# JackAILab/ConsistentID

Hardware: AMD Instinct MI355X
Metric: 512x512 SD1.5 images/sec/node @50 DDIM steps (higher is better)
Workload: dtype f16; 1 GPU; sd15 ConsistentID 512x512, 50 DDIM steps, batch 4/GPU (global 4), CFG batch 8, LoRA rank 128 merged, start_merge_step 30, hipGraph on; global_batch=4, parallelism=dp1 (images sharded, no in-step collective)

## Files before the change

### consistentid_amd/csrc/gemm.hip

```cpp
#include "xattn_core.h"
#include "gemm_args.h"
#include "../../include/cid.h"

#ifndef CID_HALO_STAGGER
#define CID_HALO_STAGGER 1
#endif
#ifdef CID_CONV_TRACE
__device__ unsigned long long g_conv_trace[2 * 4096];
#define CONV_STAMP(k) do { if (tr_on) tr_ts[k] = __builtin_readcyclecounter(); } while (0)
#define CONV_FLUSH() do { if (tr_on && lane == 0 && tr_n + 8 <= 4096) { for (int q_ = 0; q_ < 8; ++q_) g_conv_trace[tr_slot * 4096 + tr_n + q_] = tr_ts[q_]; } tr_n += 8; } while (0)
#else
#define CONV_STAMP(k) do { } while (0)
#define CONV_FLUSH() do { } while (0)
#endif
#if defined(CID_GEMM_ABLATION)
#define CID_ABL(bit) ((a.ablate & (bit)) != 0)
#else
#define CID_ABL(bit) false
#endif

namespace {
using cidg::GemmArgs;
using cidg::wait_vmcnt;

template <int N>
__device__ __forceinline__ void frags_landed(half8 (&f)[N]) {
#pragma unroll
    for (int i = 0; i < N; ++i) asm volatile("" : "+v"(f[i]));
}


constexpr int BK = 64;

typedef float f32x4v __attribute__((ext_vector_type(4)));

CID_DEVINL f32x4v mfma16(half8 a, half8 b, f32x4v c) {
    return __builtin_amdgcn_mfma_f32_16x16x32_f16(a, b, c, 0, 0, 0);
}

CID_DEVINL int swz_key(int r) { return ((r >> 1) & 3) << 1; }
CID_DEVINL int lds_off(int r, int c) { return r * 128 + ((c ^ swz_key(r)) << 4); }

CID_DEVINL float row16_sum(float v) {
#define CID_ROR(N) v += __builtin_bit_cast(float, __builtin_amdgcn_update_dpp(0, __builtin_bit_cast(int, v), 0x120 + N, 0xf, 0xf, false))
    CID_ROR(8); CID_ROR(4); CID_ROR(2); CID_ROR(1);
#undef CID_ROR
    return v;
}

template <int TM, int TN, bool VMODE, bool LN, bool NLOOP = false, bool ACT = false>
CID_DEVINL void igemm_epilogue(const GemmArgs& a, f32x4v (&acc)[TM][TN], int m0, int n0, int wm, int wn,
                               int l16, int lq, char* smem, int wave, const float (&lmean)[TM], const float (&lrstd)[TM],
                               int nwaves, int wn_count, const half4 (&rpre)[TM][TN], bool rpre_valid) {
    if constexpr (VMODE) {
#pragma unroll
        for (int c = 0; c < TN; ++c) {
            const int n = n0 + (wn * TN + c) * 16 + l16;
            if (n >= a.n_end) continue;
            const int cg = n - a.n_vt0;
            const int head = cg / a.dhead, dd = cg - head * a.dhead;
            const float bv = LN ? a.ln_b[n] : (a.bias ? (float)a.bias[n] : 0.f);
            const float sv = LN ? a.ln_s[n] : 0.f;
#pragma unroll
            for (int t = 0; t < TM; ++t) {
                const int mt = m0 + (wm * TM + t) * 16;
                if (mt >= a.M) continue;
                const int b = mt / a.ntok, tok0 = mt - b * a.ntok;
                half_t* dst = a.vt + ((long)(b * a.heads + head) * a.dvp + dd) * a.ntok + tok0;
                half4 o;
                if constexpr (LN) {
#pragma unroll
                    for (int i = 0; i < 4; ++i) {
                        const float mu = __shfl(lmean[t], 4 * lq + i, 64), rs = __shfl(lrstd[t], 4 * lq + i, 64);
                        o[i] = (half_t)(rs * (acc[t][c][i] - mu * sv) + bv);
                    }
                } else {
#pragma unroll
                    for (int i = 0; i < 4; ++i) o[i] = (half_t)(acc[t][c][i] + bv);
                }
                *reinterpret_cast<half4*>(dst + 8 * (lq & 1) + 4 * (lq >> 1)) = o;
            }
        }
        return;
    } else {
        if (!NLOOP && a.splitk > 1) {
            float* wsp = a.ws + (long)blockIdx.z * a.M * a.N;
#pragma unroll
            for (int t = 0; t < TM; ++t) {
                const int m = m0 + (wm * TM + t) * 16 + l16;
                if (m >= a.M) continue;
#pragma unroll
                for (int c = 0; c < TN; ++c) {
                    const int n = n0 + (wn * TN + c) * 16 + 4 * lq;
                    if (n >= a.n_end) continue;
                    *reinterpret_cast<f32x4v*>(wsp + (long)m * a.N + n) = acc[t][c];
                }
            }
            return;
        }
        if (NLOOP || a.mode == 1) {
#pragma unroll
            for (int c = 0; c + 1 < TN; c += 2) {
                const int nt = n0 + (wn * TN + c) * 16;
                if (nt >= a.n_end) continue;
                float bv[4] = {0.f, 0.f, 0.f, 0.f}, bg[4] = {0.f, 0.f, 0.f, 0.f};
                float sv[4] = {0.f, 0.f, 0.f, 0.f}, sg[4] = {0.f, 0.f, 0.f, 0.f};
                if constexpr (LN) {
                    const f32x4v fv = *reinterpret_cast<const f32x4v*>(a.ln_b + nt + 4 * lq);
                    const f32x4v fg = *reinterpret_cast<const f32x4v*>(a.ln_b + nt + 16 + 4 * lq);
                    const f32x4v qv = *reinterpret_cast<const f32x4v*>(a.ln_s + nt + 4 * lq);
                    const f32x4v qg = *reinterpret_cast<const f32x4v*>(a.ln_s + nt + 16 + 4 * lq);
#pragma unroll
                    for (int i = 0; i < 4; ++i) { bv[i] = fv[i]; bg[i] = fg[i]; sv[i] = qv[i]; sg[i] = qg[i]; }
                } else if (a.bias && !CID_ABL(512)) {
                    const half4 hv = *reinterpret_cast<const half4*>(a.bias + nt + 4 * lq);
                    const half4 hg = *reinterpret_cast<const half4*>(a.bias + nt + 16 + 4 * lq);
// ... 78 lines not shown
                }
                if constexpr (ACT) {
#pragma unroll
                    for (int i = 0; i < 4; ++i) v[i] = __builtin_fmaxf(v[i], 0.f);
                }
                half4 o;
#pragma unroll
                for (int i = 0; i < 4; ++i) o[i] = (half_t)v[i];
                *reinterpret_cast<half4*>(stg + (t * 16 + l16) * P + c * 16 + 4 * lq) = o;
                if (gstat && mok) {
#pragma unroll
                    for (int i = 0; i < 4; ++i) { const float f = (float)o[i]; gs[c][i] += f; gq[c][i] = __builtin_fmaf(f, f, gq[c][i]); }
                }
            }
        }
        float* gst = reinterpret_cast<float*>(smem + nwaves * (TM * 16 * P) * 2);
        if (gstat) {
#pragma unroll
            for (int c = 0; c < TN; ++c)
#pragma unroll
                for (int i = 0; i < 4; ++i) { gs[c][i] = row16_sum(gs[c][i]); gq[c][i] = row16_sum(gq[c][i]); }
            if (l16 == 0) {
#pragma unroll
                for (int c = 0; c < TN; ++c)
#pragma unroll
                    for (int i = 0; i < 4; ++i) {
                        float* p = gst + (wave * (TN * 16) + c * 16 + 4 * lq + i) * 2;
                        p[0] = gs[c][i]; p[1] = gq[c][i];
                    }
            }
        }
        asm volatile("s_waitcnt lgkmcnt(0)" ::: "memory");
        constexpr int CPR = TN * 2;
        constexpr int PER = TM * 16 * CPR / 64;
        static_assert((TM * 16 * CPR) % 64 == 0, "tile chunks must divide over the wave");
        const int lane = lq * 16 + l16;
#pragma unroll
        for (int i = 0; i < PER; ++i) {
            const int e = i * 64 + lane;
            const int r = e / CPR, ch = e - r * CPR;
            const int m = m0 + wm * TM * 16 + r;
            const int n = n0 + wn * TN * 16 + ch * 8;
            const half8 val = *reinterpret_cast<const half8*>(stg + r * P + ch * 8);
            if (m < a.M && n < a.n_end) {
                *reinterpret_cast<half8*>(a.out + (long)m * a.ldo + n) = val;
                if (a.out2) *reinterpret_cast<half8*>(a.out2 + (long)m * a.ldo + n) = val;
            }
        }
        if (gstat) {
            __builtin_amdgcn_s_barrier();
            const int bn = wn_count * TN * 16, wm_count = nwaves / wn_count;
            const int nu = bn / a.gn_unit;
            const int u = wave * 64 + lq * 16 + l16;
            if (u < nu && n0 + u * a.gn_unit < a.n_end) {
                float S = 0.f, Q = 0.f;
                for (int w_ = 0; w_ < wm_count; ++w_)
                    for (int ch = u * a.gn_unit; ch < (u + 1) * a.gn_unit; ++ch) {
                        const int wv = w_ * wn_count + ch / (TN * 16);
                        const float* p = gst + (wv * (TN * 16) + ch % (TN * 16)) * 2;
                        S += p[0]; Q += p[1];
                    }
                float* dst = a.gn_stats + ((long)(m0 / (wm_count * TM * 16)) * (a.N / a.gn_unit) + (n0 - a.n_begin) / a.gn_unit + u) * 2;
                dst[0] = S; dst[1] = Q;
            }
        }
    }
}

template <int TM, int TN>
CID_DEVINL bool prefetch_residual(const GemmArgs& a, half4 (&rpre)[TM][TN], int m0, int n0, int wm, int wn, int l16, int lq) {
    const bool on = TM >= 4 && a.res != nullptr && a.mode == 0 && a.splitk == 1;
    if constexpr (TM < 4) return false;
#pragma unroll
    for (int t = 0; t < TM; ++t)
#pragma unroll
        for (int c = 0; c < TN; ++c) {
            const int m = m0 + (wm * TM + t) * 16 + l16, n = n0 + (wn * TN + c) * 16 + 4 * lq;
            half4 z = {(half_t)0.f, (half_t)0.f, (half_t)0.f, (half_t)0.f};
            rpre[t][c] = (on && m < a.M && n < a.n_end) ? *reinterpret_cast<const half4*>(a.res + (long)m * a.ldr + n) : z;
        }
    return on;
}

template <int TM, int TN, int WM, int WN, bool VMODE, int NBUF, bool LN, bool NLOOP = false, int ATT_D = 0, bool ACT = false>
__global__ void __launch_bounds__(64 * WM * WN, (NLOOP && TM == 2) ? 4 : 2)
igemm_kernel(GemmArgs a) {
#if defined(__HIP_DEVICE_COMPILE__)
    constexpr int NW = WM * WN;
    constexpr int BM = 16 * TM * WM;
    constexpr int BN = 16 * TN * WN;
    constexpr int XPW = (BM / 8 + NW - 1) / NW, WPW = (BN / 8 + NW - 1) / NW;
    constexpr int XI = XPW * NW, WI = WPW * NW;
    constexpr int XBYTES = XI * 1024, WBYTES = BN * 128;
    constexpr int SBYTES = XBYTES + WBYTES;
    extern __shared__ __attribute__((aligned(16))) char smem[];
    typedef __attribute__((address_space(3))) void lds_void;

    const int tid = threadIdx.x;
    const int lane = tid & 63;
    const int wave = __builtin_amdgcn_readfirstlane(tid >> 6);
    const int l16 = lane & 15, lq = lane >> 4;
    const int r8 = lane >> 3, c8 = lane & 7;
    const int wm = wave / WN, wn = wave % WN;
    int nb_, mb_;
    cidg::xcd_tile(a, nb_, mb_);
    const int n0 = a.n_begin + nb_ * BN * a.nloop;
    const int m0 = mb_ * BM;

    constexpr unsigned OOB = 0x80000000u;
    const __amdgpu_buffer_rsrc_t rs_x1 = __builtin_amdgcn_make_buffer_rsrc((void*)a.x1, 0, a.bytes_x1, 0x00020000);
    const __amdgpu_buffer_rsrc_t rs_x2 = __builtin_amdgcn_make_buffer_rsrc((void*)(a.x2 ? a.x2 : a.x1), 0,
                                                                           a.x2 ? a.bytes_x2 : 0, 0x00020000);
    const __amdgpu_buffer_rsrc_t rs_w = __builtin_amdgcn_make_buffer_rsrc((void*)a.w, 0, a.bytes_w, 0x00020000);
    int xb[XPW], xy[XPW], xx[XPW], xsw[XPW];
    bool xok[XPW];
#pragma unroll
    for (int j = 0; j < XPW; ++j) {
        const int R = (j * NW + wave) * 8 + r8;
        const int m = m0 + R;
        xok[j] = (R < BM) && (m < a.M);
        xsw[j] = (c8 ^ swz_key(R)) * 8;
        if (a.taps == 9) {
            const int hw = a.Ho * a.Wo;
            const int b = m / hw, rem = m - b * hw;
            xb[j] = b; xy[j] = rem / a.Wo; xx[j] = rem - xy[j] * a.Wo;
        } else {
            xb[j] = 0; xy[j] = 0; xx[j] = m;
        }
    }
    unsigned woff[WPW];
#pragma unroll
    for (int j = 0; j < WPW; ++j) {
        const int R = (j * NW + wave) * 8 + r8;
        const bool ok = (R < BN) && (n0 + R < a.n_end);
        woff[j] = ok ? (unsigned)(((long)(n0 + R) * a.ktot + (c8 ^ swz_key(R)) * 8) * 2) : OOB;
    }
    unsigned xoff1[XPW], xoff2[XPW];
    auto set_tap = [&](int tap) {
        const int dy = (a.taps == 9) ? tap / 3 + a.tap0 : 0;
        const int dx = (a.taps == 9) ? tap - (tap / 3) * 3 + a.tap0 : 0;
#pragma unroll
        for (int j = 0; j < XPW; ++j) {
            bool ok = xok[j];
            long row = xx[j];
            if (a.taps == 9) {
                int yy = xy[j] * a.stride + dy, xs = xx[j] * a.stride + dx;
                const int Hv = a.Hi << a.up, Wv = a.Wi << a.up;
                ok = ok && (yy >= 0) && (yy < Hv) && (xs >= 0) && (xs < Wv);
                yy >>= a.up; xs >>= a.up;
                row = ((long)xb[j] * a.Hi + yy) * a.Wi + xs;
            }
            xoff1[j] = ok ? (unsigned)((row * a.ld1 + xsw[j]) * 2) : OOB;
            xoff2[j] = ok ? (unsigned)((row * a.ld2 + xsw[j]) * 2) : OOB;
        }
    };
    int ld_tap = -1;

    auto issue = [&](int slab, int buf, unsigned wtile = 0u) {
        const int cs = slab / a.taps;
        const int tap = slab - cs * a.taps;
        const int cbase = cs * BK;
        if (tap != ld_tap) { set_tap(tap); ld_tap = tap; }
        char* xs = smem + buf * SBYTES;
        char* ws = xs + XBYTES;
        const bool first = cbase < a.c1;
        const unsigned coff = (unsigned)((first ? cbase : cbase - a.c1) * 2);
        if (first) {
#pragma unroll
            for (int j = 0; j < XPW; ++j)
                __builtin_amdgcn_raw_ptr_buffer_load_lds(rs_x1, (lds_void*)(xs + (j * NW + wave) * 1024), 16, xoff1[j] + coff, 0, 0, 0);
        } else {
#pragma unroll
            for (int j = 0; j < XPW; ++j)
                __builtin_amdgcn_raw_ptr_buffer_load_lds(rs_x2, (lds_void*)(xs + (j * NW + wave) * 1024), 16, xoff2[j] + coff, 0, 0, 0);
        }
        const unsigned koff = (unsigned)((tap * (a.c1 + a.c2) + cbase) * 2) + wtile;
#pragma unroll
        for (int j = 0; j < WPW; ++j)
            if ((j + 1) * NW * 8 <= BN || (j * NW + wave) * 8 < BN)
                __builtin_amdgcn_raw_ptr_buffer_load_lds(rs_w, (lds_void*)(ws + (j * NW + wave) * 1024), 16, woff[j] + koff, 0, 0, 0);
    };

    f32x4v acc[TM][TN];
#pragma unroll
    for (int t = 0; t < TM; ++t)
#pragma unroll
        for (int c = 0; c < TN; ++c) acc[t][c] = f32x4v{0.f, 0.f, 0.f, 0.f};

    const int s_begin = (int)((long)a.nslab * blockIdx.z / a.splitk);
    const int s_end = (int)((long)a.nslab * (blockIdx.z + 1) / a.splitk);

    static_assert(NBUF >= 2 && NBUF <= 4, "two to four LDS stages");
    auto read_frags = [&](const char* xs, const char* ws, int ks, half8 (&xf)[TM], half8 (&wf)[TN]) {
        if (CID_ABL(256)) return;
#pragma unroll
        for (int t = 0; t < TM; ++t)
            xf[t] = *reinterpret_cast<const half8*>(xs + lds_off((wm * TM + t) * 16 + l16, ks * 4 + lq));
#pragma unroll
        for (int c = 0; c < TN; ++c)
            wf[c] = *reinterpret_cast<const half8*>(ws + lds_off((wn * TN + c) * 16 + l16, ks * 4 + lq));
    };
    auto mma = [&](const half8 (&xf)[TM], const half8 (&wf)[TN]) {
#pragma unroll
        for (int t = 0; t < TM; ++t)
#pragma unroll
            for (int c = 0; c < TN; ++c)
                acc[t][c] = VMODE ? mfma16(xf[t], wf[c], acc[t][c]) : mfma16(wf[c], xf[t], acc[t][c]);
    };

    float lsum[TM], lsq[TM];
    half2v lpiv[TM];
#pragma unroll
    for (int t = 0; t < TM; ++t) {
        lsum[t] = 0.f; lsq[t] = 0.f;
        half_t p = (half_t)0.f;
        if constexpr (LN) {
            const int row = m0 + (wm * TM + t) * 16 + l16;
            if (row < a.M) p = a.x1[(long)row * a.ld1];
        }
        lpiv[t] = half2v{p, p};
    }
    bool ln_on = true;
    auto ln_acc = [&](const half8 (&xf)[TM]) {
        if constexpr (LN) {
            if (!ln_on) return;
            const half2v one = {(half_t)1.f, (half_t)1.f};
#pragma unroll
            for (int t = 0; t < TM; ++t)
#pragma unroll
                for (int j = 0; j < 4; ++j) {
                    const half2v h = half2v{xf[t][2 * j], xf[t][2 * j + 1]} - lpiv[t];
                    lsum[t] = __builtin_amdgcn_fdot2(h, one, lsum[t], false);
                    lsq[t] = __builtin_amdgcn_fdot2(h, h, lsq[t], false);
                }
        }
    };

    float lmean[TM], lrstd[TM];
    auto ln_finish = [&]() {
#pragma unroll
        for (int t = 0; t < TM; ++t) {
            if constexpr (LN) {
                float sm = lsum[t], sq = lsq[t];
                sm += __shfl_xor(sm, 16, 64); sq += __shfl_xor(sq, 16, 64);
                sm += __shfl_xor(sm, 32, 64); sq += __shfl_xor(sq, 32, 64);
                const float inv = 1.f / (float)a.ktot;
                const float md = sm * inv;
                lmean[t] = (float)lpiv[t][0] + md;
                lrstd[t] = sq == 0.f ? 0.f : rsqrtf(fmaxf(sq * inv - md * md, 0.f) + a.ln_eps);
            } else { lmean[t] = 0.f; lrstd[t] = 1.f; }
        }
    };

    half4 rpre[TM][TN];
    const bool rpre_valid = VMODE ? false : prefetch_residual<TM, TN>(a, rpre, m0, n0, wm, wn, l16, lq);
    if constexpr (NLOOP) {
        static_assert(NBUF == 2, "the N-loop form runs on two stages");
        const int ns = a.nslab, T = ns * a.nloop;
        const unsigned wstep = (unsigned)((long)BN * a.ktot * 2);
        int is_ks = 0; unsigned is_w = 0u;
        set_tap(0);
        auto issue_next = [&](int buf) {
            char* xs = smem + buf * SBYTES;
            char* ws = xs + XBYTES;
            const unsigned coff = (unsigned)(is_ks * BK * 2);
#pragma unroll
            for (int j = 0; j < XPW; ++j)
                __builtin_amdgcn_raw_ptr_buffer_load_lds(rs_x1, (lds_void*)(xs + (j * NW + wave) * 1024), 16, xoff1[j] + coff, 0, 0, 0);
#pragma unroll
            for (int j = 0; j < WPW; ++j)
                __builtin_amdgcn_raw_ptr_buffer_load_lds(rs_w, (lds_void*)(ws + (j * NW + wave) * 1024), 16, woff[j] + coff + is_w, 0, 0, 0);
            if (++is_ks == ns) { is_ks = 0; is_w += wstep; }
        };
        half8 xf0[TM], wf0[TN], xf1[TM], wf1[TN];
        issue_next(0);
        asm volatile("s_waitcnt vmcnt(0)" ::: "memory");
        __builtin_amdgcn_s_barrier();
        read_frags(smem, smem + XBYTES, 0, xf0, wf0);
        if (1 < T) issue_next(1);
        frags_landed(xf0); frags_landed(wf0);
        int cur = 0, ks = 0, nt = 0;
        for (int f = 0; f < T; ++f) {
            const char* xs = smem + cur * SBYTES;
            read_frags(xs, xs + XBYTES, 1, xf1, wf1);
            mma(xf0, wf0);
            ln_acc(xf0);
            __builtin_amdgcn_sched_barrier(0);
            frags_landed(xf1); frags_landed(wf1);
            if (f + 1 < T) {
                asm volatile("s_waitcnt vmcnt(0) lgkmcnt(0)" ::: "memory");
                __builtin_amdgcn_s_barrier();
                if (f + 2 < T) issue_next(cur);
                const char* xn = smem + (cur ^ 1) * SBYTES;
                read_frags(xn, xn + XBYTES, 0, xf0, wf0);
            }
            mma(xf1, wf1);
            ln_acc(xf1);
            __builtin_amdgcn_sched_barrier(0);
            frags_landed(xf0); frags_landed(wf0);
            cur ^= 1;
            if (++ks == ns) {
                if (nt == 0) { ln_finish(); ln_on = false; }
                igemm_epilogue<TM, TN, false, LN, true>(a, acc, m0, n0 + nt * BN, wm, wn, l16, lq, smem, wave, lmean, lrstd, NW, WN, rpre, false);
#pragma unroll
                for (int t = 0; t < TM; ++t)
#pragma unroll
                    for (int c = 0; c < TN; ++c) acc[t][c] = f32x4v{0.f, 0.f, 0.f, 0.f};
                ks = 0; ++nt;
                __builtin_amdgcn_sched_barrier(0);
            }
        }
        asm volatile("s_waitcnt vmcnt(0)" ::: "memory");
        return;
    }
    {
    int pw = XPW;
#pragma unroll
    for (int j = 0; j < WPW; ++j)
        if ((j + 1) * NW * 8 <= BN || (j * NW + wave) * 8 < BN) ++pw;
    half8 xf0[TM], wf0[TN], xf1[TM], wf1[TN];
    const int nsl = s_end - s_begin;
    int pre = 0;
    if (!CID_ABL(128))
        for (; pre < NBUF - 1 && pre < nsl; ++pre) issue(s_begin + pre, pre);
    if (NBUF == 2) asm volatile("s_waitcnt vmcnt(0)" ::: "memory");
    else wait_vmcnt((pre > 0 ? pre - 1 : 0) * pw);
    __builtin_amdgcn_s_barrier();
    read_frags(smem, smem + XBYTES, 0, xf0, wf0);
    if (NBUF - 1 < nsl && !CID_ABL(1)) issue(s_begin + NBUF - 1, NBUF - 1);
    frags_landed(xf0); frags_landed(wf0);

    int cur = 0;
    for (int slab = s_begin; slab < s_end; ++slab) {
        const char* xs = smem + cur * SBYTES;
        const int nxt = (cur + 1 == NBUF) ? 0 : cur + 1;
        read_frags(xs, xs + XBYTES, 1, xf1, wf1);
        if (!CID_ABL(2)) mma(xf0, wf0);
        ln_acc(xf0);
        __builtin_amdgcn_sched_barrier(0);
        frags_landed(xf1); frags_landed(wf1);
        if (slab + 1 < s_end) {
            if (NBUF == 2) asm volatile("s_waitcnt vmcnt(0) lgkmcnt(0)" ::: "memory");
            else {
                int young = s_end - 2 - slab;
                if (young > NBUF - 2) young = NBUF - 2;
                if (young < 0 || CID_ABL(1)) young = 0;
                wait_vmcnt(young * pw);
                asm volatile("s_waitcnt lgkmcnt(0)" ::: "memory");
            }
            __builtin_amdgcn_s_barrier();
            if (slab + NBUF < s_end && !CID_ABL(1)) issue(slab + NBUF, cur);
            const char* xn = smem + nxt * SBYTES;
            read_frags(xn, xn + XBYTES, 0, xf0, wf0);
        }
        if (!CID_ABL(2)) mma(xf1, wf1);
        ln_acc(xf1);
        __builtin_amdgcn_sched_barrier(0);
        frags_landed(xf0); frags_landed(wf0);
        cur = nxt;
    }
    }
    asm volatile("s_waitcnt vmcnt(0)" ::: "memory");
    ln_finish();

    static_assert(NW * TM * 16 * (TN * 16 + 8) * 2 + NW * TN * 16 * 8 <= NBUF * SBYTES, "epilogue staging fits the pipeline stages");
    if constexpr (ATT_D > 0) {
        static_assert(!VMODE && !NLOOP && BN % ATT_D == 0 && BM % 32 == 0, "the tile spans whole heads and 32-token groups");
        constexpr int TP = BN + 8;
        static_assert(BM * TP * 2 <= NBUF * SBYTES, "the Q / O tile fits the pipeline stages");
        half_t* T = reinterpret_cast<half_t*>(smem);
        __builtin_amdgcn_s_barrier();
#pragma unroll
        for (int t = 0; t < TM; ++t)
#pragma unroll
            for (int c = 0; c < TN; ++c) {
                const int nl = (wn * TN + c) * 16 + 4 * lq;
                float v[4];
#pragma unroll
                for (int i = 0; i < 4; ++i) v[i] = acc[t][c][i];
                if constexpr (LN) {
                    const f32x4v qs = *reinterpret_cast<const f32x4v*>(a.ln_s + n0 + nl);
                    const f32x4v qb = *reinterpret_cast<const f32x4v*>(a.ln_b + n0 + nl);
#pragma unroll
                    for (int i = 0; i < 4; ++i) v[i] = lrstd[t] * (v[i] - lmean[t] * qs[i]) + qb[i];
                }
                half4 o;
#pragma unroll
                for (int i = 0; i < 4; ++i) o[i] = (half_t)v[i];
                *reinterpret_cast<half4*>(T + ((wm * TM + t) * 16 + l16) * TP + nl) = o;
            }
        asm volatile("s_waitcnt lgkmcnt(0)" ::: "memory");
        __builtin_amdgcn_s_barrier();
        {
            const int idx = lane & 31, hi = lane >> 5;
            const long row = a.att_kvrow[m0 / a.ntok];
            constexpr int QKS = (ATT_D + 15) / 16, DVT = (ATT_D + 31) / 32;
            constexpr int NHL = BN / ATT_D, NTG = BM / 32;
            const int h0 = n0 / ATT_D;
            for (int u = wave; u < NHL * NTG; u += NW) {
                const int hl = u / NTG, tg = u - hl * NTG;
                const half_t* kph = a.att_kp + row * a.att_krow + (long)(h0 + hl) * XC_KTILES * QKS * 512 + lane * 8;
                const half_t* vph = a.att_vp + row * a.att_vrow + (long)(h0 + hl) * DVT * XC_PV_KSTEPS * 512 + lane * 8;
                xattn_core_unit<ATT_D, 1, true>(T, TP, tg * 32, hl * ATT_D, kph, vph, a.att_n_txt, a.att_n_ip, a.att_scale, idx, hi);
            }
        }
        asm volatile("s_waitcnt lgkmcnt(0)" ::: "memory");
        __builtin_amdgcn_s_barrier();
        constexpr int CPR = BN / 8;
        for (int e = tid; e < BM * CPR; e += 64 * NW) {
            const int r = e / CPR, cc = e - r * CPR;
            if (m0 + r < a.M)
                *reinterpret_cast<half8*>(a.out + (long)(m0 + r) * a.ldo + n0 + cc * 8) = *reinterpret_cast<const half8*>(T + r * TP + cc * 8);
        }
        return;
    }
    igemm_epilogue<TM, TN, VMODE, LN, false, ACT>(a, acc, m0, n0, wm, wn, l16, lq, smem, wave, lmean, lrstd, NW, WN, rpre, rpre_valid);
#endif
}

template <int TM, int TN, int WM, int WN>
__global__ void __launch_bounds__(64 * WM * WN, 2)
igemm_halo_kernel(GemmArgs a) {
#if defined(__HIP_DEVICE_COMPILE__)
    constexpr int NW = WM * WN;
    constexpr int BM = 16 * TM * WM;
    constexpr int BN = 16 * TN * WN;
    constexpr int HPW = 7;
    constexpr int HROWS = HPW * NW * 8;
    constexpr int WPW = (BN / 8 + NW - 1) / NW;
    constexpr int HBYTES = HROWS * 128, WBYTES = WPW * NW * 1024;
    extern __shared__ __attribute__((aligned(16))) char smem[];
    typedef __attribute__((address_space(3))) void lds_void;
    char* hbuf = smem;
    char* wbuf = smem + 2 * HBYTES;

    const int tid = threadIdx.x;
    const int lane = tid & 63;
    const int wave = __builtin_amdgcn_readfirstlane(tid >> 6);
    const int l16 = lane & 15, lq = lane >> 4;
    const int r8 = lane >> 3, c8 = lane & 7;
    const int wm = wave / WN, wn = wave % WN;
    int nb_, mb_;
    cidg::xcd_tile(a, nb_, mb_);
    const int n0 = a.n_begin + nb_ * BN;
    const int m0 = mb_ * BM;

    const int W = a.Wo, H = a.Ho, HW = H * W;
    const int seg_tok = BM < HW ? BM : HW;
    const int rs = seg_tok / W;
    const int hs = (rs + 2) * (W + 2);
    const int nh = (BM / seg_tok) * hs;
    const int img0 = m0 / HW;
    const int y0 = (m0 - img0 * HW) / W;

    constexpr unsigned OOB = 0x80000000u;
    const __amdgpu_buffer_rsrc_t rs_x1 = __builtin_amdgcn_make_buffer_rsrc((void*)a.x1, 0, a.bytes_x1, 0x00020000);
    const __amdgpu_buffer_rsrc_t rs_x2 = __builtin_amdgcn_make_buffer_rsrc((void*)(a.x2 ? a.x2 : a.x1), 0,
                                                                           a.x2 ? a.bytes_x2 : 0, 0x00020000);
    const __amdgpu_buffer_rsrc_t rs_w = __builtin_amdgcn_make_buffer_rsrc((void*)a.w, 0, a.bytes_w, 0x00020000);

    unsigned hoff1[HPW], hoff2[HPW];
#pragma unroll
    for (int j = 0; j < HPW; ++j) {
        const int hr = (j * NW + wave) * 8 + r8;
        const int seg = hr / hs, rem = hr - seg * hs;
        const int hy = rem / (W + 2), hx = rem - hy * (W + 2);
        const int img = img0 + seg;
        const int yy = y0 + hy - 1, xx = hx - 1;
        const bool ok = (hr < nh) && (yy >= 0) && (yy < H) && (xx >= 0) && (xx < W) && ((long)img * HW < a.M);
        const long row = ((long)img * H + yy) * W + xx;
        const int swz = (c8 ^ swz_key(hr)) * 8;
        hoff1[j] = ok ? (unsigned)((row * a.ld1 + swz) * 2) : OOB;
        hoff2[j] = ok ? (unsigned)((row * a.ld2 + swz) * 2) : OOB;
    }
    unsigned woff[WPW];
#pragma unroll
    for (int j = 0; j < WPW; ++j) {
        const int R = (j * NW + wave) * 8 + r8;
        const bool ok = (R < BN) && (n0 + R < a.n_end);
        woff[j] = ok ? (unsigned)(((long)(n0 + R) * a.ktot + (c8 ^ swz_key(R)) * 8) * 2) : OOB;
    }
    int hbase[TM];
#pragma unroll
    for (int t = 0; t < TM; ++t) {
        const int ml = (wm * TM + t) * 16 + l16;
        const int seg = ml / seg_tok, rem = ml - seg * seg_tok;
        const int y = rem / W, x = rem - y * W;
        hbase[t] = seg * hs + (y + 1) * (W + 2) + (x + 1);
        asm volatile("" : "+v"(hbase[t]));
    }

    const int ctot = a.c1 + a.c2;
    auto issue_halo = [&](int cs, int hb) {
        const int cbase = cs * BK;
        char* dst = hbuf + hb * HBYTES;
        if (cbase < a.c1) {
#pragma unroll
            for (int j = 0; j < HPW; ++j)
                if ((j * NW + wave) * 8 < nh)
                    __builtin_amdgcn_raw_ptr_buffer_load_lds(rs_x1, (lds_void*)(dst + (j * NW + wave) * 1024), 16, hoff1[j] + cbase * 2, 0, 0, 0);
// ... 226 lines not shown
        *reinterpret_cast<half4*>(a.out + (long)m * a.ldo + n) = o;
        if (a.out2) *reinterpret_cast<half4*>(a.out2 + (long)m * a.ldo + n) = o;
    }
}

template <int TM, int TN, int WM, int WN, bool VMODE, bool LN, bool NLOOP = false, int NBUF = 2, int ATT_D = 0, bool ACT = false>
int launch_one_ln(const GemmArgs& a, int ncols, hipStream_t s) {
    constexpr int BM = 16 * TM * WM, BN = 16 * TN * WN;
    constexpr int NW = WM * WN;
    constexpr int STAGE = ((BM / 8 + NW - 1) / NW) * NW * 1024 + BN * 128;
    constexpr int SMEM = NBUF * STAGE;
    static_assert(SMEM <= 160 * 1024, "LDS budget");
    auto kern = igemm_kernel<TM, TN, WM, WN, VMODE, NBUF, LN, NLOOP, ATT_D, ACT>;
    static bool configured = false;
    if (!configured) {
        hipError_t herr = hipFuncSetAttribute((const void*)kern, hipFuncAttributeMaxDynamicSharedMemorySize, SMEM);
        if (herr != hipSuccess) {
            cid_set_error("cid_gemm_f16: cannot reserve %d bytes of LDS (%s)", SMEM, hipGetErrorString(herr));
            return -5;
        }
        configured = true;
    }
    dim3 grid((ncols + BN - 1) / BN / (NLOOP ? a.nloop : 1), (a.M + BM - 1) / BM, VMODE ? 1 : a.splitk);
    GemmArgs b = a;
    b.xcd_pn = cidg::choose_xcd_pn((int)grid.x, (int)grid.y, 2.0 * ncols * a.ktot, (double)a.bytes_x1 + a.bytes_x2);
    hipLaunchKernelGGL(kern, grid, dim3(64 * WM * WN), SMEM, s, b);
    return 0;
}

template <int TM, int TN, int WM, int WN, bool VMODE>
int launch_one(const GemmArgs& a, int ncols, hipStream_t s) {
    if constexpr (!VMODE && TN == 4 && WM * WN == 8) {
        if (a.nloop > 1)
            return a.ln_s ? launch_one_ln<TM, TN, WM, WN, false, true, true>(a, ncols, s)
                          : launch_one_ln<TM, TN, WM, WN, false, false, true>(a, ncols, s);
    }
    if constexpr (!VMODE && TN == 5) {
        if (a.nbuf == 3)
            return a.ln_s ? launch_one_ln<TM, TN, WM, WN, false, true, false, 3>(a, ncols, s)
                          : launch_one_ln<TM, TN, WM, WN, false, false, false, 3>(a, ncols, s);
    }
    return a.ln_s ? launch_one_ln<TM, TN, WM, WN, VMODE, true>(a, ncols, s) : launch_one_ln<TM, TN, WM, WN, VMODE, false>(a, ncols, s);
}

template <int TM, int TN, int WM, int WN, int ATT_D>
int launch_att(const GemmArgs& a, hipStream_t s) {
    return a.ln_s ? launch_one_ln<TM, TN, WM, WN, false, true, false, 2, ATT_D>(a, a.N, s)
                  : launch_one_ln<TM, TN, WM, WN, false, false, false, 2, ATT_D>(a, a.N, s);
}

template <int TM, int TN, int WM, int WN>
int launch_act(const GemmArgs& a, hipStream_t s) {
    return launch_one_ln<TM, TN, WM, WN, false, false, false, 2, 0, true>(a, a.N, s);
}

void launch_splitk_epilogue(const GemmArgs& a, hipStream_t s) {
    const long items = (long)a.M * (a.N >> 2);
    const int grid = (int)((items + 255) / 256 > 2048 ? 2048 : (items + 255) / 256);
    hipLaunchKernelGGL(splitk_epilogue_kernel, dim3(grid), dim3(256), 0, s, a);
}

template <int TM, int TN, int WM, int WN>
int launch_halo(GemmArgs a, hipStream_t s) {
    constexpr int BM = 16 * TM * WM, BN = 16 * TN * WN, NW = WM * WN;
    constexpr int SMEM = 2 * (7 * NW * 1024) + 2 * (((BN / 8 + NW - 1) / NW) * NW * 1024);
    static_assert(SMEM <= 160 * 1024, "LDS budget");
    auto kern = igemm_halo_kernel<TM, TN, WM, WN>;
    static bool configured = false;
    if (!configured) {
        hipError_t herr = hipFuncSetAttribute((const void*)kern, hipFuncAttributeMaxDynamicSharedMemorySize, SMEM);
        if (herr != hipSuccess) {
            cid_set_error("cid_gemm_f16: cannot reserve %d bytes of LDS (%s)", SMEM, hipGetErrorString(herr));
            return -5;
        }
        configured = true;
    }
    dim3 grid((a.N + BN - 1) / BN, (a.M + BM - 1) / BM, a.splitk);
    a.xcd_pn = cidg::choose_xcd_pn((int)grid.x, (int)grid.y, 2.0 * a.N * a.ktot, (double)a.bytes_x1 + a.bytes_x2);
    hipLaunchKernelGGL(kern, grid, dim3(64 * NW), SMEM, s, a);
    if (a.splitk > 1) launch_splitk_epilogue(a, s);
    return 0;
}

template <int TM, int TN, int WM, int WN>
int launch(GemmArgs a, hipStream_t s) {
    const int n_plain = (a.mode == 2) ? a.n_vt0 : a.N;
    a.n_begin = 0; a.n_end = n_plain;
    int rc = launch_one<TM, TN, WM, WN, false>(a, n_plain, s);
    if (rc) return rc;
    if (a.splitk > 1) launch_splitk_epilogue(a, s);
    if (a.mode == 2 && a.N > a.n_vt0) {
        GemmArgs v = a;
        v.n_begin = a.n_vt0; v.n_end = a.N; v.splitk = 1;
        rc = launch_one<TM, TN, WM, WN, true>(v, a.N - a.n_vt0, s);
    }
    return rc;
}

}

extern "C" int cid_gemm_f16(const cid_gemm_desc* d, cid_stream_t stream) {
    using namespace cidg;
    GemmPlan p;
    int rc = plan(d, p);
    if (rc) return rc;
    const GemmArgs& a = p.a;
    hipStream_t s = (hipStream_t)stream;
    switch (p.family) {
        case CID_GEMM_FAMILY_GEGLU_H32:
            rc = launch_geglu_h32(a, s);
            break;
        case CID_GEMM_FAMILY_IGEMM_ATT:
            if (p.cfg == G128x128) rc = launch_att<2, 4, 4, 2, 64>(a, s);
            else if (p.cfg == B128x160) rc = a.dhead == 80 ? launch_att<2, 5, 4, 2, 80>(a, s) : launch_att<2, 5, 4, 2, 160>(a, s);
            else rc = a.dhead == 80 ? launch_att<2, 5, 2, 2, 80>(a, s) : launch_att<2, 5, 2, 2, 160>(a, s);
            break;
        case CID_GEMM_FAMILY_CONV_H32:
        case CID_GEMM_FAMILY_CONV_H32_PHASE:
            rc = launch_conv_h32(a, p.bm, s);
            break;
        case CID_GEMM_FAMILY_IGEMM_HALO:
            rc = launch_halo<4, 5, 4, 2>(a, s);
            break;
        default:
            if (p.act) {
                switch (p.cfg) {
                    case A256x160: rc = launch_act<4, 5, 4, 2>(a, s); break;
                    case B128x160: rc = launch_act<2, 5, 4, 2>(a, s); break;
                    case C64x160:  rc = launch_act<2, 5, 2, 2>(a, s); break;
                    case G256x128: rc = launch_act<4, 4, 4, 2>(a, s); break;
                    case G128x128: rc = launch_act<2, 4, 4, 2>(a, s); break;
                    case O64x64:   rc = launch_act<2, 2, 2, 2>(a, s); break;
                    case O128x32:  rc = launch_act<2, 2, 4, 1>(a, s); break;
                }
            } else {
                switch (p.cfg) {
                    case A256x160: rc = launch<4, 5, 4, 2>(a, s); break;
                    case B128x160: rc = launch<2, 5, 4, 2>(a, s); break;
                    case C64x160:  rc = launch<2, 5, 2, 2>(a, s); break;
                    case G256x128: rc = launch<4, 4, 4, 2>(a, s); break;
                    case G128x128: rc = launch<2, 4, 4, 2>(a, s); break;
                    case O64x64:   rc = launch<2, 2, 2, 2>(a, s); break;
                    case O128x32:  rc = launch<2, 2, 4, 1>(a, s); break;
                }
            }
            break;
    }
    if (rc) return rc;
    CID_CHECK_LAUNCH("cid_gemm_f16");
    return 0;
}
```

### consistentid_amd/csrc/gemm_args.h

```cpp
#pragma once
#include "common.h"

struct cid_gemm_desc;

namespace cidg {

struct GemmArgs {
    const half_t* x1; const half_t* x2;
    int c1, c2, ld1, ld2;
    const half_t* w;
    half_t* out; int ldo;
    half_t* out2;
    const half_t* bias;
    const half_t* rowbias; int ld_rowbias; int rows_per_sample;
    const half_t* res; int ldr;
    int M, N, taps;
    int Hi, Wi, Ho, Wo, stride, up;
    int mode;
    half_t* vt; int n_vt0, heads, dhead, dvp, ntok;
    int n_begin, n_end;
    int ktot;
    int nslab;
    int cslabs;
    int splitk;
    int nloop;
    int nbuf;
    const half_t* att_kp; const half_t* att_vp; const int* att_kvrow;
    long att_krow, att_vrow;
    int att_n_txt, att_n_ip;
    float att_scale;
    unsigned bytes_x1, bytes_x2, bytes_w;
    float* ws;
    const float* ln_s;
    const float* ln_b;
    float ln_eps;
    float* gn_stats;
    int gn_unit;
    int ablate;
    int xcd_pn;
    int tap0;
    const half_t* w4;
};

CID_DEVINL void xcd_tile(const GemmArgs& a, int& nb, int& mb) {
    const int gx = gridDim.x, gy = gridDim.y;
    int bid = blockIdx.y * gx + blockIdx.x;
    if (a.xcd_pn > 0) {
        const int pn = a.xcd_pn;
        const int x = bid & 7, l = bid >> 3;
        const int bnc = gx / pn;
        nb = (x % pn) * bnc + l % bnc;
        mb = (x / pn) * (gy * pn >> 3) + l / bnc;
    } else {
        const int nwg = gx * gy;
        if ((nwg & 7) == 0) bid = (bid & 7) * (nwg >> 3) + (bid >> 3);
        nb = bid % gx;
        mb = bid / gx;
    }
}

int choose_xcd_pn(int gx, int gy, double w_bytes, double x_bytes);

enum TileCfg { A256x160, B128x160, C64x160, G256x128, G128x128, O64x64, O128x32 };
struct GemmPlan {
    GemmArgs a;
    TileCfg cfg;
    int bm, bn;
    int family;
    bool ln, act, vmode;
    bool sk_epilogue;
    int stats_rows;
};
int plan(const cid_gemm_desc* d, GemmPlan& p);

CID_DEVINL void wait_vmcnt(int n) {
#define CID_VM(N) case N: asm volatile("s_waitcnt vmcnt(" #N ")" ::: "memory"); break;
    switch (n) {
        CID_VM(0) CID_VM(1) CID_VM(2) CID_VM(3) CID_VM(4) CID_VM(5) CID_VM(6) CID_VM(7) CID_VM(8) CID_VM(9)
        CID_VM(10) CID_VM(11) CID_VM(12) CID_VM(13) CID_VM(14) CID_VM(15) CID_VM(16) CID_VM(17) CID_VM(18)
        CID_VM(19) CID_VM(20) CID_VM(21) CID_VM(22) CID_VM(23) CID_VM(24) CID_VM(25) CID_VM(26) CID_VM(27)
        CID_VM(28) CID_VM(29) CID_VM(30) CID_VM(31) CID_VM(32)
        default: asm volatile("s_waitcnt vmcnt(0)" ::: "memory"); break;
    }
#undef CID_VM
}

int launch_conv_h32(const GemmArgs& a, int bm, hipStream_t s);

int launch_geglu_h32(const GemmArgs& a, hipStream_t s);

}
```

### consistentid_amd/csrc/gemm_plan.hip

```cpp
#include "gemm_args.h"
#include "../../include/cid.h"
#include <stdlib.h>

namespace {
using namespace cidg;

int env_int(const char* name, int dflt) { const char* e = getenv(name); return e ? atoi(e) : dflt; }

struct PlanSwitches {
    int geglu_tile = env_int("CID_GEGLU_TILE", 0);
    int gemm_tile = env_int("CID_GEMM_TILE", 0);
    int gemm_sk = env_int("CID_GEMM_SK", 0);
    int prefer128 = env_int("CID_GEMM_PREFER128", 1);
    int geglu_nloop = env_int("CID_GEGLU_NLOOP", 0);
    int geglu_h32 = env_int("CID_GEGLU_H32", 1);
    int nbuf = env_int("CID_GEMM_NBUF", 0);
    int no_halo = env_int("CID_GEMM_NOHALO", 0);
    int conv_h32 = env_int("CID_CONV_H32", 1);
    int upconv_fold = env_int("CID_UPCONV_FOLD", 1);
    int xcd_2d = env_int("CID_XCD_2D", 1);
    int ablate = env_int("CID_GEMM_ABLATE", 0);
};

const PlanSwitches& switches() { static const PlanSwitches s; return s; }

constexpr int BK = 64;
constexpr long TARGET = 2048;

void set_tile(GemmPlan& p, TileCfg cfg) {
    static const int bm[] = { 256, 128, 64, 256, 128, 64, 128 }, bn[] = { 160, 160, 160, 128, 128, 64, 32 };
    p.cfg = cfg; p.bm = bm[cfg]; p.bn = bn[cfg];
}

int n_plain(const cid_gemm_desc* d) { return d->mode == 2 ? d->n_vt0 : d->N; }

long waves(const cid_gemm_desc* d, int bm, int bn, int w) { return (long)((d->M + bm - 1) / bm) * ((n_plain(d) + bn - 1) / bn) * w; }

int check_args(const cid_gemm_desc* d, GemmPlan& p) {
    CID_CHECK_ARG(d && d->x1 && d->w && d->out, "cid_gemm_f16: null pointer");
    CID_CHECK_ARG(d->taps == 1 || d->taps == 9, "cid_gemm_f16: taps must be 1 or 9 (got %d)", d->taps);
    CID_CHECK_ARG(d->c1 > 0 && d->c1 % 32 == 0 && d->c2 >= 0 && d->c2 % 32 == 0 && (d->c1 + d->c2) % 64 == 0 &&
                  (d->c2 == 0 || d->c1 % 64 == 0),
                  "cid_gemm_f16: channel counts must be multiples of 64 (c1=%d c2=%d)", d->c1, d->c2);
    CID_CHECK_ARG(d->c2 == 0 || d->x2, "cid_gemm_f16: c2 > 0 needs x2");
    CID_CHECK_ARG(d->N > 0 && d->N % 32 == 0 && d->M > 0, "cid_gemm_f16: bad M/N (%d, %d)", d->M, d->N);
    CID_CHECK_ARG(d->mode >= 0 && d->mode <= 3, "cid_gemm_f16: bad mode %d", d->mode);
    CID_CHECK_ARG(d->ld1 % 8 == 0 && d->ldo % 8 == 0 && (d->c2 == 0 || d->ld2 % 8 == 0) && (!d->res || d->ldr % 8 == 0),
                  "cid_gemm_f16: row pitches (ld1, ld2, ldo, ldr) must keep 16-byte alignment");
    CID_CHECK_ARG((((uintptr_t)d->out | (uintptr_t)d->res | (uintptr_t)d->out2) & 15) == 0,
                  "cid_gemm_f16: out / out2 / res must be 16-byte aligned (rows are stored and the residual is read in 16-byte chunks)");
    CID_CHECK_ARG((d->ln_s == nullptr) == (d->ln_b == nullptr), "cid_gemm_f16: ln_s and ln_b come together");
    CID_CHECK_ARG(!d->ln_s || (d->taps == 1 && d->c2 == 0 && !d->bias && d->ln_eps > 0.f),
                  "cid_gemm_f16: the LayerNorm fold applies to one-source linears; the bias belongs in ln_b");
    CID_CHECK_ARG(!d->out2 || d->mode == 0, "cid_gemm_f16: out2 (a second destination) goes with the plain epilogue, mode 0");
    const long rows_in = (d->taps == 9) ? (long)(d->M / (d->Ho * d->Wo)) * d->Hi * d->Wi : (long)d->M;
    const long b1 = ((rows_in - 1) * d->ld1 + d->c1) * 2, b2 = d->c2 ? ((rows_in - 1) * d->ld2 + d->c2) * 2 : 0;
    const long bw = (long)d->N * d->taps * (d->c1 + d->c2) * 2;
    CID_CHECK_ARG(b1 < 0x7fffffffL && b2 < 0x7fffffffL && bw < 0x7fffffffL, "cid_gemm_f16: tensor exceeds 2 GiB");
    p.a.bytes_x1 = (unsigned)b1; p.a.bytes_x2 = (unsigned)b2; p.a.bytes_w = (unsigned)bw;
    if (d->taps == 9) {
        CID_CHECK_ARG(d->Hi > 0 && d->Wi > 0 && d->Ho > 0 && d->Wo > 0 && (d->stride == 1 || d->stride == 2)
                      && (d->up == 0 || d->up == 1), "cid_gemm_f16: bad conv geometry");
        CID_CHECK_ARG(d->M % (d->Ho * d->Wo) == 0, "cid_gemm_f16: M is not batch * Ho * Wo");
    }
    CID_CHECK_ARG(d->pad_mode == 0 || d->pad_mode == 1, "cid_gemm_f16: bad pad_mode %d", d->pad_mode);
    CID_CHECK_ARG(d->pad_mode == 0 || (d->mode == 0 && d->taps == 9 && d->stride == 2 && d->up == 0 && d->Hi % 2 == 0 &&
                                       d->Wi % 2 == 0 && d->Ho == d->Hi / 2 && d->Wo == d->Wi / 2),
                  "cid_gemm_f16: pad_mode 1 needs mode 0, taps 9, stride 2, up 0, even Hi / Wi, Ho = Hi / 2 and Wo = Wi / 2 "
                  "(got mode %d taps %d stride %d up %d, %d x %d -> %d x %d)", d->mode, d->taps, d->stride, d->up, d->Hi, d->Wi,
                  d->Ho, d->Wo);
    CID_CHECK_ARG(!d->w_up4 || (d->taps == 9 && d->up == 1 && d->stride == 1 && d->mode == 0 && !d->res),
                  "cid_gemm_f16: w_up4 needs taps 9, up 1, stride 1, mode 0 and no res (got taps %d up %d stride %d mode %d)",
                  d->taps, d->up, d->stride, d->mode);
    CID_CHECK_ARG(((uintptr_t)d->w_up4 & 15) == 0, "cid_gemm_f16: w_up4 must be 16-byte aligned");
    CID_CHECK_ARG(d->act == 0 || d->act == 1, "cid_gemm_f16: bad act %d", d->act);
    CID_CHECK_ARG(d->act == 0 || (d->mode == 0 && !d->gn_stats && !d->ws && !d->ln_s),
                  "cid_gemm_f16: act 1 needs mode 0 and no gn_stats / ws / ln_s (got mode %d)", d->mode);
    return 0;
}

void fill_args(const cid_gemm_desc* d, GemmPlan& p) {
    GemmArgs& a = p.a;
    a.x1 = (const half_t*)d->x1; a.x2 = (const half_t*)d->x2;
    a.c1 = d->c1; a.c2 = d->c2; a.ld1 = d->ld1; a.ld2 = d->ld2;
    a.w = (const half_t*)d->w; a.out = (half_t*)d->out; a.ldo = d->ldo;
    a.out2 = (half_t*)d->out2;
    a.bias = (const half_t*)d->bias;
    a.rowbias = (const half_t*)d->rowbias; a.ld_rowbias = d->ld_rowbias;
    a.rows_per_sample = d->rows_per_sample > 0 ? d->rows_per_sample : 1;
    a.res = (const half_t*)d->res; a.ldr = d->ldr;
    a.M = d->M; a.N = d->N; a.taps = d->taps;
    a.Hi = d->Hi; a.Wi = d->Wi; a.Ho = d->Ho; a.Wo = d->Wo; a.stride = d->stride; a.up = d->up;
    a.mode = d->mode;
    a.vt = (half_t*)d->vt; a.n_vt0 = d->n_vt0; a.heads = d->heads; a.dhead = d->dhead;
    a.dvp = d->dvp; a.ntok = d->ntok;
    a.cslabs = (d->c1 + d->c2) / BK;
    a.ktot = d->taps * (d->c1 + d->c2);
    a.nslab = a.ktot / BK;
    a.splitk = 1; a.nloop = 1; a.nbuf = 2; a.xcd_pn = 0;
    a.att_kp = (const half_t*)d->att_kp; a.att_vp = (const half_t*)d->att_vp; a.att_kvrow = (const int*)d->att_kvrow;
    a.att_n_txt = d->att_n_txt; a.att_n_ip = d->att_n_ip; a.att_scale = d->att_ip_scale;
    a.att_krow = a.att_vrow = 0;
    a.ws = (float*)d->ws;
// ... 149 lines not shown
}

void route_conv3x3(const cid_gemm_desc* d, GemmPlan& p) {
    GemmArgs& a = p.a;
    const bool only256 = switches().conv_h32 == 2;
    const int HW = d->taps == 9 ? d->Ho * d->Wo : 0;
    const bool shape_ok = switches().conv_h32 != 0 && !d->act && d->mode == 0 && d->taps == 9 && d->stride == 1 && (d->up == 0 || d->up == 1) &&
                          d->Wo == (d->Wi << d->up) && d->Ho == (d->Hi << d->up) && d->N % 160 == 0 && HW >= 64 &&
                          (!d->rowbias || (a.rows_per_sample >= 64 && a.rows_per_sample % 64 == 0));
    const bool fold_ok = shape_ok && switches().upconv_fold && d->w_up4 && d->up == 1 && d->c2 == 0 && !d->rowbias && !d->res &&
                         (long)d->N * d->c1 * 32 < 0x7fffffffL;
    for (int bm_try = 256; shape_ok && bm_try >= (only256 ? 256 : 128); bm_try >>= 1) {
        const long tiles = (long)(d->M / bm_try) * (d->N / 160);
        if (tiles < 256 || (bm_try == 128 && a.cslabs > 10) || d->M % bm_try != 0) continue;
        if (fold_ok && (d->Hi * d->Wi) % bm_try == 0 && bm_try % d->Wi == 0 && (bm_try / d->Wi + 2) * (d->Wi + 2) <= 400)
            a.w4 = (const half_t*)d->w_up4;
        else {
            const int seg = bm_try < HW ? bm_try : HW;
            if (seg % d->Wo != 0 || HW % seg != 0 || bm_try % seg != 0) continue;
            if (d->up && (seg != bm_try || (seg / d->Wo) % 2 != 0)) continue;
            const int nh = (bm_try / seg) * (((seg / d->Wo) >> d->up) + 2) * ((d->Wo >> d->up) + 2);
            if (nh > 400) continue;
        }
        p.family = a.w4 ? CID_GEMM_FAMILY_CONV_H32_PHASE : CID_GEMM_FAMILY_CONV_H32;
        p.bm = bm_try;
        a.splitk = 1;
        return;
    }
}

void finish_launch(const cid_gemm_desc* d, GemmPlan& p) {
    const int f = p.family;
    const bool plain = f == CID_GEMM_FAMILY_IGEMM && !d->act;
    if (f == CID_GEMM_FAMILY_GEGLU_H32) p.bn = 160;
    p.act = f == CID_GEMM_FAMILY_IGEMM && d->act;
    p.ln = (plain || f == CID_GEMM_FAMILY_IGEMM_ATT) && p.a.ln_s != nullptr;
    p.vmode = plain && p.a.mode == 2 && p.a.N > p.a.n_vt0;
    p.sk_epilogue = (plain || f == CID_GEMM_FAMILY_IGEMM_HALO) && p.a.splitk > 1;
    if (f != CID_GEMM_FAMILY_IGEMM && f != CID_GEMM_FAMILY_IGEMM_ATT) p.a.nbuf = 0;
}

int check_stats(const cid_gemm_desc* d, GemmPlan& p) {
    const int unit = d->N / 32;
    const bool ok = d->mode == 0 && d->act == 0 && p.a.splitk == 1 && (p.cfg == A256x160 || p.cfg == B128x160 || p.cfg == C64x160) &&
                    d->N % 32 == 0 && unit > 0 && 80 % unit == 0 && p.bm > 0 && d->M % p.bm == 0;
    p.stats_rows = ok ? p.bm : 0;
    CID_CHECK_ARG(!p.a.gn_stats || p.stats_rows > 0,
                  "cid_gemm_f16: gn_stats requested for a launch that cannot emit them (ask cid_gemm_stats_rows first)");
    return 0;
}

}

int cidg::plan(const cid_gemm_desc* d, GemmPlan& p) {
    if (int rc = check_args(d, p)) return rc;
    fill_args(d, p);
    if (d->mode == 3) {
        if (int rc = tiles_mode3(d, p)) return rc;
    } else {
        if (int rc = choose_tiles(d, p)) return rc;
        plan_nloop(d, p);
        route_linear_h32(d, p);
        plan_ring(d, p);
        route_halo(d, p);
        route_conv3x3(d, p);
    }
    finish_launch(d, p);
    return check_stats(d, p);
}

int cidg::choose_xcd_pn(int gx, int gy, double w_bytes, double x_bytes) {
    if (!switches().xcd_2d || ((long)gx * gy) % 8 != 0) return 0;
    int best = 0;
    double cost = 0.0;
    for (int pn = 1; pn <= 8; pn *= 2) {
        const int pm = 8 / pn;
        if (gx % pn != 0 || gy % pm != 0) continue;
        const double c = pm * w_bytes + pn * x_bytes;
        if (best == 0 || c < cost) { best = pn; cost = c; }
    }
    return best;
}

extern "C" int cid_gemm_plan(const cid_gemm_desc* d, cid_gemm_plan_info* out) {
    CID_CHECK_ARG(out, "cid_gemm_plan: null output");
    cidg::GemmPlan p;
    int rc = cidg::plan(d, p);
    if (rc) return rc;
    out->family = p.family; out->bm = p.bm; out->bn = p.bn;
    out->splitk = p.a.splitk; out->nloop = p.a.nloop; out->nbuf = p.a.nbuf;
    out->ln = p.ln; out->act = p.act; out->vmode = p.vmode;
    out->splitk_epilogue = p.sk_epilogue; out->stats_rows = p.stats_rows;
    return 0;
}

extern "C" int cid_gemm_stats_rows(const cid_gemm_desc* d) {
    if (!d) return 0;
    cid_gemm_desc q = *d;
    q.gn_stats = nullptr;
    cidg::GemmPlan p;
    return cidg::plan(&q, p) == 0 ? p.stats_rows : 0;
}
```

Baseline: 7.752 images/s.

## Fuse QKV projection's plain and V-transposed parts into a single launch

Mode-2 GEMMs (QKV projection, where V is written transposed) were launched as two kernels, one for the plain Q/K columns and one for the V columns. A new merged kernel covers the whole N range in one grid. Each workgroup picks the MFMA operand order and epilogue at runtime from whether its column tile lies in the V region, and tiles are interleaved so Q/K and V tiles are spread across the grid. This removes a launch and a tail, and lets V tiles share the activation reads. The cost is a runtime branch, larger code, and a remapped tile order that may change cache locality.

```diff
diff --git a/consistentid_amd/csrc/gemm.hip b/consistentid_amd/csrc/gemm.hip
--- a/consistentid_amd/csrc/gemm.hip
+++ b/consistentid_amd/csrc/gemm.hip
@@ -32,6 +32,8 @@
 
 constexpr int BK = 64;
 
+template <bool B> struct BoolC { static constexpr bool value = B; };
+
 typedef float f32x4v __attribute__((ext_vector_type(4)));
 
 CID_DEVINL f32x4v mfma16(half8 a, half8 b, f32x4v c) {
@@ -276,10 +278,11 @@
     return on;
 }
 
-template <int TM, int TN, int WM, int WN, bool VMODE, int NBUF, bool LN, bool NLOOP = false, int ATT_D = 0, bool ACT = false>
-__global__ void __launch_bounds__(64 * WM * WN, (NLOOP && TM == 2) ? 4 : 2)
-igemm_kernel(GemmArgs a) {
+template <int TM, int TN, int WM, int WN, bool VMODE, int NBUF, bool LN, bool NLOOP, int ATT_D, bool ACT, bool QKV>
+__device__ __forceinline__ void igemm_body(const GemmArgs& a) {
 #if defined(__HIP_DEVICE_COMPILE__)
+    constexpr bool MERGED = QKV;
+    static_assert(!MERGED || (!VMODE && !NLOOP && ATT_D == 0 && !ACT), "the one-launch QKV form is a plain instance");
     constexpr int NW = WM * WN;
     constexpr int BM = 16 * TM * WM;
     constexpr int BN = 16 * TN * WN;
@@ -298,8 +301,13 @@
     const int wm = wave / WN, wn = wave % WN;
     int nb_, mb_;
     cidg::xcd_tile(a, nb_, mb_);
+    if constexpr (MERGED) {
+        const int nq = a.n_vt0 / BN, nv = (int)gridDim.x - nq;
+        if (nq == 2 * nv) { const int g = nb_ / 3, r = nb_ - 3 * g; nb_ = (r == 2) ? nq + g : 2 * g + r; }
+    }
     const int n0 = a.n_begin + nb_ * BN * a.nloop;
     const int m0 = mb_ * BM;
+    const bool vwg = MERGED && n0 >= a.n_vt0;
 
     constexpr unsigned OOB = 0x80000000u;
     const __amdgpu_buffer_rsrc_t rs_x1 = __builtin_amdgcn_make_buffer_rsrc((void*)a.x1, 0, a.bytes_x1, 0x00020000);
@@ -394,12 +402,13 @@
         for (int c = 0; c < TN; ++c)
             wf[c] = *reinterpret_cast<const half8*>(ws + lds_off((wn * TN + c) * 16 + l16, ks * 4 + lq));
     };
-    auto mma = [&](const half8 (&xf)[TM], const half8 (&wf)[TN]) {
+    auto mma = [&](auto vtag, const half8 (&xf)[TM], const half8 (&wf)[TN]) {
+        constexpr bool V = decltype(vtag)::value;
 #pragma unroll
         for (int t = 0; t < TM; ++t)
 #pragma unroll
             for (int c = 0; c < TN; ++c)
-                acc[t][c] = VMODE ? mfma16(xf[t], wf[c], acc[t][c]) : mfma16(wf[c], xf[t], acc[t][c]);
+                acc[t][c] = V ? mfma16(xf[t], wf[c], acc[t][c]) : mfma16(wf[c], xf[t], acc[t][c]);
     };
 
     float lsum[TM], lsq[TM];
@@ -477,7 +486,7 @@
         for (int f = 0; f < T; ++f) {
             const char* xs = smem + cur * SBYTES;
             read_frags(xs, xs + XBYTES, 1, xf1, wf1);
-            mma(xf0, wf0);
+            mma(BoolC<false>{}, xf0, wf0);
             ln_acc(xf0);
             __builtin_amdgcn_sched_barrier(0);
             frags_landed(xf1); frags_landed(wf1);
@@ -488,7 +497,7 @@
                 const char* xn = smem + (cur ^ 1) * SBYTES;
                 read_frags(xn, xn + XBYTES, 0, xf0, wf0);
             }
-            mma(xf1, wf1);
+            mma(BoolC<false>{}, xf1, wf1);
             ln_acc(xf1);
             __builtin_amdgcn_sched_barrier(0);
             frags_landed(xf0); frags_landed(wf0);
@@ -507,7 +516,7 @@
         asm volatile("s_waitcnt vmcnt(0)" ::: "memory");
         return;
     }
-    {
+    auto ring = [&](auto vtag) {
     int pw = XPW;
 #pragma unroll
     for (int j = 0; j < WPW; ++j)
@@ -529,7 +538,7 @@
         const char* xs = smem + cur * SBYTES;
         const int nxt = (cur + 1 == NBUF) ? 0 : cur + 1;
         read_frags(xs, xs + XBYTES, 1, xf1, wf1);
-        if (!CID_ABL(2)) mma(xf0, wf0);
+        if (!CID_ABL(2)) mma(vtag, xf0, wf0);
         ln_acc(xf0);
         __builtin_amdgcn_sched_barrier(0);
         frags_landed(xf1); frags_landed(wf1);
@@ -547,13 +556,17 @@
             const char* xn = smem + nxt * SBYTES;
             read_frags(xn, xn + XBYTES, 0, xf0, wf0);
         }
-        if (!CID_ABL(2)) mma(xf1, wf1);
+        if (!CID_ABL(2)) mma(vtag, xf1, wf1);
         ln_acc(xf1);
         __builtin_amdgcn_sched_barrier(0);
         frags_landed(xf0); frags_landed(wf0);
         cur = nxt;
     }
-    }
+    };
+    if constexpr (MERGED) {
+        if (vwg) ring(BoolC<true>{});
+        else ring(BoolC<false>{});
+    } else ring(BoolC<VMODE>{});
     asm volatile("s_waitcnt vmcnt(0)" ::: "memory");
     ln_finish();
 
@@ -608,8 +621,26 @@
         }
         return;
     }
+    if constexpr (MERGED) {
+        if (vwg) {
+            igemm_epilogue<TM, TN, true, LN>(a, acc, m0, n0, wm, wn, l16, lq, smem, wave, lmean, lrstd, NW, WN, rpre, false);
+            return;
+        }
+    }
     igemm_epilogue<TM, TN, VMODE, LN, false, ACT>(a, acc, m0, n0, wm, wn, l16, lq, smem, wave, lmean, lrstd, NW, WN, rpre, rpre_valid);
 #endif
+}
+
+template <int TM, int TN, int WM, int WN, bool VMODE, int NBUF, bool LN, bool NLOOP = false, int ATT_D = 0, bool ACT = false>
+__global__ void __launch_bounds__(64 * WM * WN, (NLOOP && TM == 2) ? 4 : 2)
+igemm_kernel(GemmArgs a) {
+    igemm_body<TM, TN, WM, WN, VMODE, NBUF, LN, NLOOP, ATT_D, ACT, false>(a);
+}
+
+template <int TM, int TN, int WM, int WN, int NBUF, bool LN>
+__global__ void __launch_bounds__(64 * WM * WN, 2)
+igemm_qkv_kernel(GemmArgs a) {
+    igemm_body<TM, TN, WM, WN, false, NBUF, LN, false, 0, false, true>(a);
 }
 
 template <int TM, int TN, int WM, int WN>
@@ -1002,8 +1033,49 @@
     return 0;
 }
 
+template <int TM, int TN, int WM, int WN, int NBUF, bool LN>
+int launch_qkv_one(const GemmArgs& a, hipStream_t s) {
+    constexpr int BM = 16 * TM * WM, BN = 16 * TN * WN;
+    constexpr int NW = WM * WN;
+    constexpr int STAGE = ((BM / 8 + NW - 1) / NW) * NW * 1024 + BN * 128;
+    constexpr int SMEM = NBUF * STAGE;
+    static_assert(SMEM <= 160 * 1024, "LDS budget");
+    auto kern = igemm_qkv_kernel<TM, TN, WM, WN, NBUF, LN>;
+    static bool configured = false;
+    if (!configured) {
+        hipError_t herr = hipFuncSetAttribute((const void*)kern, hipFuncAttributeMaxDynamicSharedMemorySize, SMEM);
+        if (herr != hipSuccess) {
+            cid_set_error("cid_gemm_f16: cannot reserve %d bytes of LDS (%s)", SMEM, hipGetErrorString(herr));
+            return -5;
+        }
+        configured = true;
+    }
+    dim3 grid((a.N + BN - 1) / BN, (a.M + BM - 1) / BM, 1);
+    GemmArgs b = a;
+    b.n_begin = 0; b.n_end = a.N;
+    b.xcd_pn = cidg::choose_xcd_pn((int)grid.x, (int)grid.y, 2.0 * a.N * a.ktot, (double)a.bytes_x1 + a.bytes_x2);
+    hipLaunchKernelGGL(kern, grid, dim3(64 * NW), SMEM, s, b);
+    return 0;
+}
+
+template <int BN>
+bool qkv_one_launch(const GemmArgs& a) {
+    return a.mode == 2 && a.n_vt0 > 0 && a.N > a.n_vt0 && a.n_vt0 % BN == 0 && a.splitk == 1 && a.nloop == 1 && !cidg::qkv_split();
+}
+
+template <int TM, int TN, int WM, int WN>
+int launch_qkv(const GemmArgs& a, hipStream_t s) {
+    if constexpr (TN == 5) {
+        if (a.nbuf == 3) return a.ln_s ? launch_qkv_one<TM, TN, WM, WN, 3, true>(a, s) : launch_qkv_one<TM, TN, WM, WN, 3, false>(a, s);
+    }
+    return a.ln_s ? launch_qkv_one<TM, TN, WM, WN, 2, true>(a, s) : launch_qkv_one<TM, TN, WM, WN, 2, false>(a, s);
+}
+
 template <int TM, int TN, int WM, int WN>
 int launch(GemmArgs a, hipStream_t s) {
+    if constexpr (TM < 4 && TN != 4) {
+        if (qkv_one_launch<16 * TN * WN>(a)) return launch_qkv<TM, TN, WM, WN>(a, s);
+    }
     const int n_plain = (a.mode == 2) ? a.n_vt0 : a.N;
     a.n_begin = 0; a.n_end = n_plain;
     int rc = launch_one<TM, TN, WM, WN, false>(a, n_plain, s);
diff --git a/consistentid_amd/csrc/gemm_args.h b/consistentid_amd/csrc/gemm_args.h
--- a/consistentid_amd/csrc/gemm_args.h
+++ b/consistentid_amd/csrc/gemm_args.h
@@ -61,6 +61,8 @@
 
 int choose_xcd_pn(int gx, int gy, double w_bytes, double x_bytes);
 
+int qkv_split();
+
 enum TileCfg { A256x160, B128x160, C64x160, G256x128, G128x128, O64x64, O128x32 };
 struct GemmPlan {
     GemmArgs a;
diff --git a/consistentid_amd/csrc/gemm_plan.hip b/consistentid_amd/csrc/gemm_plan.hip
--- a/consistentid_amd/csrc/gemm_plan.hip
+++ b/consistentid_amd/csrc/gemm_plan.hip
@@ -19,6 +19,7 @@
     int conv_h32 = env_int("CID_CONV_H32", 1);
     int upconv_fold = env_int("CID_UPCONV_FOLD", 1);
     int xcd_2d = env_int("CID_XCD_2D", 1);
+    int qkv_split = env_int("CID_QKV_SPLIT", 0);
     int ablate = env_int("CID_GEMM_ABLATE", 0);
 };
 
@@ -334,6 +335,8 @@
     return best;
 }
 
+int cidg::qkv_split() { return switches().qkv_split; }
+
 extern "C" int cid_gemm_plan(const cid_gemm_desc* d, cid_gemm_plan_info* out) {
     CID_CHECK_ARG(out, "cid_gemm_plan: null output");
     cidg::GemmPlan p;
```

Result: no change. 7.780 images/s, median of 6 (+0.4%).
